# DSXiangLi/ChineseNER

Hardware: AMD Instinct MI355X
Metric: training samples/sec, bert_bilstm_crf (BERT-base + BiLSTM + CRF), msra-shaped (higher is better)
Workload: dtype bf16; 1 GPU; model=bert_bilstm_crf, global_batch=64, seq_len=128, parallelism=dp1

## Files before the change

### chinesener_amd/ops/functional.py

```python
from __future__ import annotations

import math
import os
from typing import Optional, Tuple

import torch
import torch.nn.functional as F

from . import reference as ref
from . import hip_enabled, get_ext


def _pad_last(t: torch.Tensor, target: int) -> torch.Tensor:
    d = t.shape[-1]
    return t if d == target else F.pad(t, (0, target - d))


class _LayerNormFn(torch.autograd.Function):
    @staticmethod
    def forward(ctx, x, weight, bias, eps):
        y, mean, rstd = get_ext().layernorm_fwd(x, weight, bias, eps)
        ctx.save_for_backward(x, weight, mean, rstd)
        return y

    @staticmethod
    def backward(ctx, dy):
        x, weight, mean, rstd = ctx.saved_tensors
        dx, dw, db = get_ext().layernorm_bwd(dy.contiguous(), x, weight, mean, rstd)
        return dx, dw, db, None


def layernorm(x, weight, bias, eps: float = 1e-12):
    if hip_enabled(x):
        shape = x.shape
        y = _LayerNormFn.apply(x.reshape(-1, shape[-1]).contiguous(), weight, bias, eps)
        return y.reshape(shape)
    return ref.layernorm(x, weight, bias, eps)


class _AddLayerNormFn(torch.autograd.Function):
    @staticmethod
    def forward(ctx, x, residual, weight, bias, eps):
        y, s, mean, rstd = get_ext().add_layernorm_fwd(x, residual, weight, bias, eps)
        ctx.save_for_backward(s, weight, mean, rstd)
        return y

    @staticmethod
    def backward(ctx, dy):
        s, weight, mean, rstd = ctx.saved_tensors
        dx, dw, db = get_ext().layernorm_bwd(dy.contiguous(), s, weight, mean, rstd)
        return dx, dx, dw, db, None


_rng_counter = None


def _rng_counter_for(device):
    global _rng_counter
    if _rng_counter is None or _rng_counter.device != device:
        seed = torch.initial_seed() & 0x7FFFFFFF
        _rng_counter = torch.tensor([seed], dtype=torch.int64, device=device)
    return _rng_counter


class _DropoutAddLNFn(torch.autograd.Function):

    @staticmethod
    def forward(ctx, x, res, weight, bias, eps, keep):
        y, s, mask, mean, rstd = get_ext().dropout_add_ln_fwd(
            x, res, weight, bias, eps, keep,
            _rng_counter_for(x.device))
        ctx.save_for_backward(s, weight, mask, mean, rstd)
        ctx.keep = keep
        return y

    @staticmethod
    def backward(ctx, dy):
        s, weight, mask, mean, rstd = ctx.saved_tensors
        dsum, dx, dw, db, _ = get_ext().dropout_add_ln_bwd(
            dy.contiguous(), s, weight, mean, rstd, mask, ctx.keep, False)
        return dx, dsum, dw, db, None, None


def dropout_add_layernorm(x, residual, weight, bias, eps: float = 1e-12,
                          p: float = 0.1, training: bool = True):
    if (training and p > 0 and hip_enabled(x) and x.dtype == torch.bfloat16
            and os.environ.get("CHINESENER_NO_FUSED_DROPOUT") != "1"):
        shape = x.shape
        y = _DropoutAddLNFn.apply(
            x.reshape(-1, shape[-1]).contiguous(),
            residual.to(x.dtype).reshape(-1, shape[-1]).contiguous(),
            weight, bias, eps, 1.0 - p)
        return y.reshape(shape)
    if training and p > 0:
        x = F.dropout(x, p, training)
    return add_layernorm(x, residual, weight, bias, eps)


def add_layernorm(x, residual, weight, bias, eps: float = 1e-12):
    if hip_enabled(x):
        shape = x.shape
        y = _AddLayerNormFn.apply(
            x.reshape(-1, shape[-1]).contiguous(),
            residual.to(x.dtype).reshape(-1, shape[-1]).contiguous(),
            weight, bias, eps)
        return y.reshape(shape)
    return ref.add_layernorm(x, residual, weight, bias, eps)


_GEMM_NT_CHOICE: dict = {}
_GEMM_NT_CALLS: dict = {}
_PICK_MIN_RECUR = 6


def _gemm_nt_mode() -> str:
    return os.environ.get("CHINESENER_GEMM_NT", "auto")


def _gemm_nt_ok(x2, w):
    return (x2.shape[0] % 128 == 0 and w.shape[0] % 128 == 0
            and w.shape[1] % 64 == 0 and x2.dtype == torch.bfloat16
            and w.dtype == torch.bfloat16)


def _tuning_active() -> bool:
    try:
        import torch.cuda.tunable as tun
        return tun.is_enabled() and tun.tuning_is_enabled()
    except Exception:
        return False


def _med_time(fn):
    import time as _time
    fn(); fn()
    torch.cuda.synchronize()
    ts = []
    for _ in range(3):
        t0 = _time.perf_counter()
        for _i in range(8):
            fn()
        torch.cuda.synchronize()
        ts.append((_time.perf_counter() - t0) / 8)
    return sorted(ts)[1]


def _pick2(key, fn_ours, fn_lib, min_recur: int = _PICK_MIN_RECUR) -> bool:
    hit = _GEMM_NT_CHOICE.get(key)
    if hit is not None:
        return hit
    if torch.cuda.is_current_stream_capturing() or _tuning_active():
        return False
    n = _GEMM_NT_CALLS.get(key, 0) + 1
    _GEMM_NT_CALLS[key] = n
    if n < min_recur:
        return False

    t_ours, t_lib = _med_time(fn_ours), _med_time(fn_lib)
    _GEMM_NT_CHOICE[key] = bool(t_ours <= t_lib)
    if os.environ.get("CHINESENER_GEMM_DEBUG") == "1":
        import sys
        print(f"[gemm-dispatch] {key}: ours {t_ours*1e6:.1f}us "
              f"lib {t_lib*1e6:.1f}us -> "
              f"{'ours' if _GEMM_NT_CHOICE[key] else 'lib'}",
              file=sys.stderr, flush=True)
    return _GEMM_NT_CHOICE[key]


def _pick_gemm_nt(x2, w, b) -> bool:
    key = (x2.shape[0], w.shape[0], w.shape[1], b is not None)
    hit = _GEMM_NT_CHOICE.get(key)
    if hit is not None:
        return hit
    if torch.cuda.is_current_stream_capturing() or _tuning_active():
        return False
    n = _GEMM_NT_CALLS.get(key, 0) + 1
    _GEMM_NT_CALLS[key] = n
    if n < _PICK_MIN_RECUR:
        return False
    ext = get_ext()

    t_ours = _med_time(lambda: ext.gemm_nt(x2, w, b, False))
    t_lib = _med_time(lambda: F.linear(x2, w, b))
    _GEMM_NT_CHOICE[key] = bool(t_ours <= t_lib)
    if os.environ.get("CHINESENER_GEMM_DEBUG") == "1":
        import sys
        print(f"[gemm-dispatch] fwd {key}: ours {t_ours*1e6:.1f}us "
              f"lib {t_lib*1e6:.1f}us -> "
              f"{'ours' if _GEMM_NT_CHOICE[key] else 'lib'}",
              file=sys.stderr, flush=True)
    return _GEMM_NT_CHOICE[key]


def _linear_fwd(x, w, b):
    mode = _gemm_nt_mode()
    if mode != "off":
        x2 = x.reshape(-1, x.shape[-1])
        if _gemm_nt_ok(x2, w):
            x2 = x2.contiguous()
            wc = w.contiguous()
            if mode == "force" or _pick_gemm_nt(x2, wc, b):
                y = get_ext().gemm_nt(x2, wc, b, False)
                return y.reshape(*x.shape[:-1], w.shape[0])
    return F.linear(x, w, b)


def _linear_dgrad(dyf, x, w):
    M, N = dyf.shape
    K = x.shape[-1]
    mode = _gemm_nt_mode()
    bf16 = (dyf.dtype == torch.bfloat16 and x.dtype == torch.bfloat16
            and w.dtype == torch.bfloat16)

    def dx_ours():
        return get_ext().gemm_nn(dyf.contiguous(), w.contiguous(), False)

    def dx_lib():
        return dyf @ w.to(dyf.dtype)

    if (mode != "off" and bf16 and M % 128 == 0 and K % 128 == 0
            and N % 64 == 0
            and (mode == "force"
                 or _pick2(("dx", M, N, K), dx_ours, dx_lib))):
        return dx_ours().reshape(x.shape)
    return dx_lib().reshape(x.shape)


def _linear_wgrad(dyf, x, w):
    M, N = dyf.shape
    K = x.shape[-1]
    x2 = x.reshape(-1, K)
    mode = _gemm_nt_mode()
    bf16 = dyf.dtype == torch.bfloat16 and x.dtype == torch.bfloat16

    def dw_ours():
        return get_ext().gemm_tn(dyf.contiguous(), x2.contiguous(), 0, False)

    def dw_lib():
        return dyf.T @ x2

    if (mode != "off" and bf16 and N % 128 == 0 and K % 128 == 0
            and M % 64 == 0
            and (mode == "force"
                 or _pick2(("dw", M, N, K), dw_ours, dw_lib))):
        return dw_ours().to(w.dtype)
    return dw_lib().to(w.dtype)


class _LinearFn(torch.autograd.Function):

    @staticmethod
    def forward(ctx, x, w, b):
        ctx.save_for_backward(x, w)
        ctx.has_bias = b is not None
        return _linear_fwd(x, w, b)

    @staticmethod
    def backward(ctx, dy):
        x, w = ctx.saved_tensors
        dyf = dy.reshape(-1, w.shape[0]).contiguous()
        dx = _linear_dgrad(dyf, x, w)
        dw = _linear_wgrad(dyf, x, w)
        db = get_ext().colsum(dyf) if ctx.has_bias else None
        return dx, dw, db


def linear(x, weight, bias=None):
    if (hip_enabled(x) and x.dtype == weight.dtype
            and not torch.is_autocast_enabled()):
        return _LinearFn.apply(x, weight,
                               bias.to(x.dtype) if bias is not None else None)
    return F.linear(x, weight, bias)


class _LinearDropoutAddLNFn(torch.autograd.Function):

    @staticmethod
    def forward(ctx, x, w, b, res, ln_w, ln_b, eps, keep):
        a = _linear_fwd(x, w, b)
        y, s, mask, mean, rstd = get_ext().dropout_add_ln_fwd(
            a.reshape(-1, a.shape[-1]).contiguous(), res, ln_w, ln_b, eps,
            keep, _rng_counter_for(x.device))
        ctx.save_for_backward(x, w, s, ln_w, mask, mean, rstd)
        ctx.keep = keep
        ctx.has_bias = b is not None
        return y

    @staticmethod
    def backward(ctx, dy):
        x, w, s, ln_w, mask, mean, rstd = ctx.saved_tensors
        dsum, dx_drop, dw_ln, db_ln, dbias = get_ext().dropout_add_ln_bwd(
            dy.contiguous(), s, ln_w, mean, rstd, mask, ctx.keep,
            ctx.has_bias)
        dx = _linear_dgrad(dx_drop, x, w)
        dw = _linear_wgrad(dx_drop, x, w)
        return dx, dw, dbias, dsum, dw_ln, db_ln, None, None


def linear_dropout_add_layernorm(x, weight, bias, residual, ln_w, ln_b,
                                 eps: float = 1e-12, p: float = 0.1,
                                 training: bool = True):
    if (training and p > 0 and hip_enabled(x) and x.dtype == torch.bfloat16
            and weight.dtype == x.dtype
            and (bias is None or bias.dtype == x.dtype)
            and os.environ.get("CHINESENER_NO_FUSED_DROPOUT") != "1"
            and not torch.is_autocast_enabled()):
        H = weight.shape[0]
        y = _LinearDropoutAddLNFn.apply(
            x, weight, bias,
            residual.to(x.dtype).reshape(-1, H).contiguous(),
            ln_w, ln_b, eps, 1.0 - p)
        return y.reshape(*x.shape[:-1], H)
    return dropout_add_layernorm(linear(x, weight, bias), residual, ln_w,
                                 ln_b, eps, p, training)


class _Embed3Fn(torch.autograd.Function):

    @staticmethod
    def forward(ctx, word_w, pos_w, tok_w, token_ids, segment_ids):
        ctx.save_for_backward(token_ids, segment_ids)
        ctx.shapes = (word_w.shape, pos_w.shape, tok_w.shape)
        return get_ext().embed3_fwd(word_w, pos_w, tok_w,
                                    token_ids.contiguous(),
                                    segment_ids.contiguous())

    @staticmethod
    def backward(ctx, dy):
        token_ids, segment_ids = ctx.saved_tensors
        (vs, ps, ts) = ctx.shapes
        B, L, H = dy.shape
        dyf = dy.reshape(-1, H).float()
        dw = torch.zeros(vs, dtype=torch.float32, device=dy.device)
        dw.index_add_(0, token_ids.reshape(-1), dyf)
        dw[0].zero_()
        dp = torch.zeros(ps, dtype=torch.float32, device=dy.device)
        dp[:L] = dy.float().sum(0)
        dt = torch.zeros(ts, dtype=torch.float32, device=dy.device)
        dt.index_add_(0, segment_ids.reshape(-1), dyf)
        return (dw.to(dy.dtype), dp.to(dy.dtype), dt.to(dy.dtype),
                None, None)


def embed3(word_w, pos_w, tok_w, token_ids, segment_ids):
    if (os.environ.get("CHINESENER_NO_EMBED3") != "1"
            and hip_enabled(word_w) and word_w.dtype == torch.bfloat16
            and word_w.shape[1] % 8 == 0
            and token_ids.shape[1] <= pos_w.shape[0]):
        return _Embed3Fn.apply(word_w, pos_w, tok_w, token_ids, segment_ids)
    pos = torch.arange(token_ids.shape[1], device=token_ids.device)
    return (F.embedding(token_ids, word_w, padding_idx=0) + pos_w[pos]
            + F.embedding(segment_ids, tok_w))


class _BiasGeluFn(torch.autograd.Function):
    @staticmethod
    def forward(ctx, x, bias):
        y = get_ext().bias_gelu_fwd(x, bias)
        ctx.save_for_backward(x, bias)
        return y

    @staticmethod
    def backward(ctx, dy):
        x, bias = ctx.saved_tensors
        dx, dbias = get_ext().bias_gelu_bwd(dy.contiguous(), x, bias)
        return dx, dbias


def bias_gelu(x, bias):
    if bias is not None and hip_enabled(x):
        shape = x.shape
        y = _BiasGeluFn.apply(x.reshape(-1, shape[-1]).contiguous(), bias)
        return y.reshape(shape)
    return ref.bias_gelu(x, bias)


def _fused_gelu_mode() -> str:
    return os.environ.get("CHINESENER_FUSED_GELU", "auto")


def _inner_decided(key) -> bool:
    return _gemm_nt_mode() != "auto" or key in _GEMM_NT_CHOICE


def _pick_fused(key, inner_key, fn_fused, fn_pair) -> bool:
    mode = _fused_gelu_mode()
    if mode != "auto":
        return mode == "force"
    if key not in _GEMM_NT_CHOICE and not _inner_decided(inner_key):
        return False
    return _pick2(key, fn_fused, fn_pair, min_recur=1)


def _ffn_up(x2, w1, b1, save_pre: bool):
    ext = get_ext()
    M, K = x2.shape
    N = w1.shape[0]

    def fused():
        return ext.gemm_nt_bias_gelu(x2, w1, b1, save_pre)

    def pair():
        u = _linear_fwd(x2, w1, None)
        return u, ext.bias_gelu_fwd(u, b1)

    key = ("ffn_up_gelu" if save_pre else "ffn_up_gelu_nopre", M, N, K)
    if _pick_fused(key, (M, N, K, False), fused, pair):
        u, g = fused()
        return u, g
    return pair()


def _ffn_dn(dx_drop, w2, u, b1):
    ext = get_ext()
    M, N = dx_drop.shape
    K = w2.shape[1]

    def fused():
        return ext.gemm_nn_dgelu(dx_drop, w2, u, b1)

    def pair():
        return ext.bias_gelu_bwd(_linear_dgrad(dx_drop, u, w2), u, b1)

    if _pick_fused(("ffn_dn_dgelu", M, N, K), ("dx", M, N, K), fused, pair):
        du, db1 = fused()
        return du, db1
    du, db1 = pair()
    return du, db1


class _FfnGeluFn(torch.autograd.Function):

    @staticmethod
    def forward(ctx, x, w1, b1, w2, b2, res, ln_w, ln_b, eps, keep):
        x2 = x.reshape(-1, x.shape[-1])
        u, g = _ffn_up(x2, w1, b1, True)
        a = _linear_fwd(g, w2, b2)
        y, s, mask, mean, rstd = get_ext().dropout_add_ln_fwd(
            a, res, ln_w, ln_b, eps, keep, _rng_counter_for(x.device))
        ctx.save_for_backward(x, w1, b1, w2, u, g, s, ln_w, mask, mean, rstd)
        ctx.keep = keep
        ctx.has_bias = b2 is not None
        return y

    @staticmethod
    def backward(ctx, dy):
        x, w1, b1, w2, u, g, s, ln_w, mask, mean, rstd = ctx.saved_tensors
        dsum, dx_drop, dw_ln, db_ln, db2 = get_ext().dropout_add_ln_bwd(
            dy.contiguous(), s, ln_w, mean, rstd, mask, ctx.keep,
            ctx.has_bias)
        dw2 = _linear_wgrad(dx_drop, g, w2)
        du, db1 = _ffn_dn(dx_drop, w2, u, b1)
        dw1 = _linear_wgrad(du, x, w1)
        dx = _linear_dgrad(du, x, w1)
        return dx, dw1, db1, dw2, db2, dsum, dw_ln, db_ln, None, None


def _ffn_fusable(x, w1, b1, w2, b2) -> bool:
    if not (hip_enabled(x) and _fused_gelu_mode() != "off"
            and not torch.is_autocast_enabled()):
        return False
    M = x.numel() // x.shape[-1] if x.shape[-1] else 0
    return (x.dtype == torch.bfloat16 and w1.dtype == x.dtype
            and w2.dtype == x.dtype and x.is_contiguous()
            and w1.is_contiguous() and w2.is_contiguous()
            and b1 is not None and b1.is_contiguous()
            and b1.dtype in (torch.bfloat16, torch.float32)
            and (b2 is None or b2.dtype == x.dtype)
            and M > 0 and M % 128 == 0 and w1.shape[0] % 128 == 0
            and w1.shape[1] % 128 == 0 and w2.shape[0] == w1.shape[1]
            and w2.shape[1] == w1.shape[0])


def ffn_gelu_dropout_add_layernorm(x, w1, b1, w2, b2, residual, ln_w, ln_b,
                                   eps: float = 1e-12, p: float = 0.1,
                                   training: bool = True):
    if _ffn_fusable(x, w1, b1, w2, b2):
        if (training and p > 0 and torch.is_grad_enabled()
                and os.environ.get("CHINESENER_NO_FUSED_DROPOUT") != "1"):
            H = w2.shape[0]
            y = _FfnGeluFn.apply(
                x, w1, b1, w2, b2,
                residual.to(x.dtype).reshape(-1, H).contiguous(),
                ln_w, ln_b, eps, 1.0 - p)
            return y.reshape(*x.shape[:-1], H)
        if not torch.is_grad_enabled():
            _, f = _ffn_up(x.reshape(-1, x.shape[-1]), w1, b1, False)
            return linear_dropout_add_layernorm(
                f.reshape(*x.shape[:-1], w1.shape[0]), w2, b2, residual,
                ln_w, ln_b, eps, p, training)
    f = bias_gelu(linear(x, w1), b1)
    return linear_dropout_add_layernorm(f, w2, b2, residual, ln_w, ln_b,
                                        eps, p, training)


def _attn_path(L: int, D: int, dtype, on_gpu: bool) -> str:
    if not on_gpu or dtype != torch.bfloat16 or D > 64 or L < 1:
        return "torch"
    mode = os.environ.get("CHINESENER_ATTN_TILED", "")
    if mode == "force":
        return "tiled" if L <= 512 else "torch"
    if ((L + 31) // 32) * 32 <= 176:
        return "lds"
    if mode != "off" and L <= 512:
        return "tiled"
    return "torch"


class _AttentionFn(torch.autograd.Function):
    @staticmethod
    def forward(ctx, q, k, v, lens, scale, tiled=False):
        ext = get_ext()
        fwd = ext.attn_tiled_fwd if tiled else ext.attn_fwd
        out, lse = fwd(q, k, v, lens, scale, 1.0, None)
        ctx.save_for_backward(q, k, v, out, lse, lens)
        ctx.scale = scale
        ctx.tiled = tiled
        return out

    @staticmethod
    def backward(ctx, dout):
        q, k, v, out, lse, lens = ctx.saved_tensors
        ext = get_ext()
        bwd = ext.attn_tiled_bwd if ctx.tiled else ext.attn_bwd
        dq, dk, dv = bwd(dout.contiguous(), q, k, v, out, lse, lens,
                         ctx.scale, 1.0, None)
        return dq, dk, dv, None, None, None


def attention(q, k, v, mask: Optional[torch.Tensor] = None,
              scale: Optional[float] = None, lens: Optional[torch.Tensor] = None):
    D = q.shape[-1]
    if scale is None:
        scale = 1.0 / math.sqrt(D)
    path = _attn_path(q.shape[2], D, q.dtype, hip_enabled(q))
    if path != "torch":
        Dp = 32 if D <= 32 else 64
        if lens is None:
            lens = (mask.long().sum(1) if mask is not None
                    else torch.full((q.shape[0],), q.shape[2],
                                    dtype=torch.long, device=q.device))
        out = _AttentionFn.apply(_pad_last(q, Dp).contiguous(),
                                 _pad_last(k, Dp).contiguous(),
                                 _pad_last(v, Dp).contiguous(),
                                 lens.to(torch.int32), float(scale),
                                 path == "tiled")
        return out[..., :D] if Dp != D else out
    return ref.attention(q, k, v, mask, scale)


class _AttentionQkvFn(torch.autograd.Function):

    @staticmethod
    def forward(ctx, qkv, lens, scale, keep, tiled=False):
        seed = None
        if keep < 1.0:
            ctr = _rng_counter_for(qkv.device)
            seed = ctr.clone()
            get_ext().bump_counter(ctr)
        ext = get_ext()
        fwd = ext.attn_tiled_fwd_qkv if tiled else ext.attn_fwd_qkv
        out, lse = fwd(qkv, lens, scale, keep, seed)
        ctx.save_for_backward(qkv, out, lse, lens,
                              seed if seed is not None
                              else torch.zeros(0))
        ctx.scale = scale
        ctx.keep = keep
        ctx.tiled = tiled
        return out

    @staticmethod
    def backward(ctx, dout):
        qkv, out, lse, lens, seed = ctx.saved_tensors
        ext = get_ext()
        bwd = ext.attn_tiled_bwd_qkv if ctx.tiled else ext.attn_bwd_qkv
        (dqkv,) = bwd(dout.contiguous(), qkv, out, lse, lens, ctx.scale,
                      ctx.keep, seed if seed.numel() else None)
        return dqkv, None, None, None, None


def attention_qkv(qkv, mask: Optional[torch.Tensor] = None,
                  lens: Optional[torch.Tensor] = None,
                  scale: Optional[float] = None,
                  p_drop: float = 0.0, training: bool = False):
    B, L, _, H, D = qkv.shape
    if scale is None:
        scale = 1.0 / math.sqrt(D)
    keep = 1.0 - p_drop if (training and p_drop > 0) else 1.0
    if os.environ.get("CHINESENER_NO_ATTN_DROP") == "1":
        keep = 1.0
    path = (_attn_path(L, D, qkv.dtype, hip_enabled(qkv))
            if D in (32, 64) else "torch")
    if path != "torch":
        if lens is None:
            lens = (mask.long().sum(1) if mask is not None
                    else torch.full((B,), L, dtype=torch.long,
                                    device=qkv.device))
        return _AttentionQkvFn.apply(qkv.contiguous(), lens.to(torch.int32),
                                     float(scale), float(keep),
                                     path == "tiled")
    q, k, v = (qkv[:, :, i].transpose(1, 2) for i in range(3))
    if keep < 1.0:
        out = ref.attention(q, k, v, mask, scale, p_drop=p_drop,
                            training=training)
    else:
        out = attention(q, k, v, mask=mask, scale=scale, lens=lens)
    return out.transpose(1, 2)


class _LinearAttentionQkvFn(torch.autograd.Function):

    @staticmethod
    def forward(ctx, x, w, b, lens, n_heads, scale, keep):
        B, L = x.shape[0], x.shape[1]
        qkv = _linear_fwd(x, w, b).reshape(B, L, 3, n_heads, -1).contiguous()
        seed = None
        if keep < 1.0:
            ctr = _rng_counter_for(x.device)
            seed = ctr.clone()
            get_ext().bump_counter(ctr)
        out, lse = get_ext().attn_fwd_qkv(qkv, lens, scale, keep, seed)
        ctx.save_for_backward(x, w, b, qkv, out, lse, lens,
                              seed if seed is not None else torch.zeros(0))
        ctx.scale = scale
        ctx.keep = keep
        return out

    @staticmethod
    def backward(ctx, dout):
        x, w, b, qkv, out, lse, lens, seed = ctx.saved_tensors
        dqkv, dbias = get_ext().attn_bwd_qkv_dbias(
            dout.contiguous(), qkv, out, lse, lens, ctx.scale, ctx.keep,
            seed if seed.numel() else None, b)
        dyf = dqkv.reshape(-1, w.shape[0])
        dx = _linear_dgrad(dyf, x, w)
        dw = _linear_wgrad(dyf, x, w)
        return dx, dw, dbias, None, None, None, None


def linear_attention_qkv(x, weight, bias, n_heads: int,
                         mask: Optional[torch.Tensor] = None,
                         lens: Optional[torch.Tensor] = None,
                         p_drop: float = 0.0, training: bool = False):
    B, L = x.shape[0], x.shape[1]
# ... 326 lines not shown
```

### csrc/bindings.cpp

```cpp
#include <torch/extension.h>

#include <vector>

std::vector<at::Tensor> layernorm_fwd(const at::Tensor&, const at::Tensor&,
                                      const at::Tensor&, double);
std::vector<at::Tensor> add_layernorm_fwd(const at::Tensor&, const at::Tensor&,
                                          const at::Tensor&, const at::Tensor&,
                                          double);
std::vector<at::Tensor> layernorm_bwd(const at::Tensor&, const at::Tensor&,
                                      const at::Tensor&, const at::Tensor&,
                                      const at::Tensor&);
at::Tensor bias_gelu_fwd(const at::Tensor&, const at::Tensor&);
std::vector<at::Tensor> bias_gelu_bwd(const at::Tensor&, const at::Tensor&,
                                      const at::Tensor&);
std::vector<at::Tensor> masked_ce_fwd(const at::Tensor&, const at::Tensor&,
                                      const at::Tensor&);
at::Tensor masked_ce_bwd(const at::Tensor&, const at::Tensor&,
                         const at::Tensor&, const at::Tensor&,
                         const at::Tensor&);
at::Tensor colsum(const at::Tensor&);
std::vector<at::Tensor> dropout_add_ln_fwd(const at::Tensor&,
                                           const at::Tensor&,
                                           const at::Tensor&,
                                           const at::Tensor&, double, double,
                                           const at::Tensor&);
at::Tensor mask_scale(const at::Tensor&, const at::Tensor&, double);
std::vector<at::Tensor> dropout_add_ln_bwd(const at::Tensor&,
                                           const at::Tensor&,
                                           const at::Tensor&,
                                           const at::Tensor&,
                                           const at::Tensor&,
                                           const at::Tensor&, double, bool);
void bump_counter(const at::Tensor&);
at::Tensor wgrad(const at::Tensor&, const at::Tensor&, long);
at::Tensor wgrad2(const at::Tensor&, const at::Tensor&, long);
at::Tensor gemm_nt(const at::Tensor&, const at::Tensor&,
                   c10::optional<at::Tensor>, bool);
at::Tensor gemm_tn(const at::Tensor&, const at::Tensor&, long, bool);
at::Tensor gemm_nn(const at::Tensor&, const at::Tensor&, bool);
std::vector<at::Tensor> gemm_nt_bias_gelu(const at::Tensor&,
                                          const at::Tensor&,
                                          const at::Tensor&, bool);
std::vector<at::Tensor> gemm_nn_dgelu(const at::Tensor&, const at::Tensor&,
                                      const at::Tensor&, const at::Tensor&);
at::Tensor embed3_fwd(const at::Tensor&, const at::Tensor&,
                      const at::Tensor&, const at::Tensor&,
                      const at::Tensor&);
std::vector<at::Tensor> crf_fwd(const at::Tensor&, const at::Tensor&,
                                const at::Tensor&, const at::Tensor&);
at::Tensor crf_viterbi(const at::Tensor&, const at::Tensor&,
                       const at::Tensor&);
std::vector<at::Tensor> crf_wide_fwd(const at::Tensor&, const at::Tensor&,
                                     const at::Tensor&, const at::Tensor&);
at::Tensor crf_wide_viterbi(const at::Tensor&, const at::Tensor&,
                            const at::Tensor&);
std::vector<at::Tensor> crf_path_posterior(const at::Tensor&,
                                           const at::Tensor&,
                                           const at::Tensor&,
                                           const at::Tensor&);
std::vector<at::Tensor> crf_nbest(const at::Tensor&, const at::Tensor&,
                                  const at::Tensor&, int64_t);
std::vector<int64_t> crf_nbest_route(int64_t, int64_t, int64_t);
at::Tensor softlexicon_fwd(const at::Tensor&, const at::Tensor&,
                           const at::Tensor&);
std::vector<at::Tensor> softlexicon_bwd(const at::Tensor&, const at::Tensor&,
                                        const at::Tensor&, const at::Tensor&);
void multi_tensor_adamw(std::vector<at::Tensor>, std::vector<at::Tensor>,
                        std::vector<at::Tensor>, std::vector<at::Tensor>,
                        std::vector<at::Tensor>, std::vector<double>,
                        std::vector<double>, double, double, double,
                        c10::optional<at::Tensor>);
at::Tensor multi_tensor_sumsq(std::vector<at::Tensor>);
void multi_tensor_scale(std::vector<at::Tensor>, const at::Tensor&);
std::vector<at::Tensor> adamw_build_meta(
    std::vector<at::Tensor>, std::vector<at::Tensor>, std::vector<at::Tensor>,
    std::vector<at::Tensor>, std::vector<at::Tensor>, std::vector<double>,
    std::vector<double>);
void multi_tensor_adamw_run(const at::Tensor&, long, long, bool, double,
                            double, double, c10::optional<at::Tensor>);
std::vector<at::Tensor> norm_build_meta(std::vector<at::Tensor>);
at::Tensor multi_tensor_sumsq_run(const at::Tensor&, long, const at::Tensor&);
void multi_tensor_scale_run(const at::Tensor&, long, const at::Tensor&);
void multi_tensor_adamw_tab_run(const at::Tensor&, long, long, bool,
                                std::vector<at::Tensor>,
                                std::vector<c10::optional<at::Tensor>>, double,
                                double, double, c10::optional<at::Tensor>,
                                c10::optional<at::Tensor>);
long grad_table_slots();
long sumsq_chunk_elems();
at::Tensor sumsq_build_chunks(std::vector<long>, std::vector<long>,
                              const at::Tensor&);
at::Tensor multi_tensor_sumsq_coef_run(const at::Tensor&, std::vector<long>,
                                       std::vector<long>,
                                       std::vector<c10::optional<at::Tensor>>,
                                       double);
std::vector<at::Tensor> attn_fwd(const at::Tensor&, const at::Tensor&,
                                 const at::Tensor&, const at::Tensor&, double,
                                 double, c10::optional<at::Tensor>);
std::vector<at::Tensor> attn_bwd(const at::Tensor&, const at::Tensor&,
                                 const at::Tensor&, const at::Tensor&,
                                 const at::Tensor&, const at::Tensor&,
                                 const at::Tensor&, double, double,
                                 c10::optional<at::Tensor>);
std::vector<at::Tensor> attn_fwd_qkv(const at::Tensor&, const at::Tensor&,
                                     double, double,
                                     c10::optional<at::Tensor>);
std::vector<at::Tensor> attn_bwd_qkv(const at::Tensor&, const at::Tensor&,
                                     const at::Tensor&, const at::Tensor&,
                                     const at::Tensor&, double, double,
                                     c10::optional<at::Tensor>);
std::vector<at::Tensor> attn_bwd_qkv_dbias(
    const at::Tensor&, const at::Tensor&, const at::Tensor&,
    const at::Tensor&, const at::Tensor&, double, double,
    c10::optional<at::Tensor>, const at::Tensor&);
std::vector<at::Tensor> attn_tiled_fwd(const at::Tensor&, const at::Tensor&,
                                       const at::Tensor&, const at::Tensor&,
                                       double, double,
                                       c10::optional<at::Tensor>);
std::vector<at::Tensor> attn_tiled_bwd(const at::Tensor&, const at::Tensor&,
                                       const at::Tensor&, const at::Tensor&,
                                       const at::Tensor&, const at::Tensor&,
                                       const at::Tensor&, double, double,
                                       c10::optional<at::Tensor>);
std::vector<at::Tensor> attn_tiled_fwd_qkv(const at::Tensor&,
                                           const at::Tensor&, double, double,
                                           c10::optional<at::Tensor>);
std::vector<at::Tensor> attn_tiled_bwd_qkv(const at::Tensor&,
                                           const at::Tensor&,
                                           const at::Tensor&,
                                           const at::Tensor&,
                                           const at::Tensor&, double, double,
                                           c10::optional<at::Tensor>);
std::vector<at::Tensor> tener_attn_fwd(const at::Tensor&, const at::Tensor&,
                                       const at::Tensor&, const at::Tensor&,
                                       const at::Tensor&, const at::Tensor&);
std::vector<at::Tensor> tener_attn_bwd(const at::Tensor&, const at::Tensor&,
                                       const at::Tensor&, const at::Tensor&,
                                       const at::Tensor&, const at::Tensor&,
                                       const at::Tensor&, const at::Tensor&,
                                       const at::Tensor&);
at::Tensor mfma_probe(const at::Tensor&, const at::Tensor&);
std::vector<at::Tensor> lstm_fwd(const at::Tensor&, const at::Tensor&,
                                 const at::Tensor&, bool, bool);
std::vector<at::Tensor> lstm_bwd(const at::Tensor&, const at::Tensor&,
                                 const at::Tensor&, const at::Tensor&,
                                 const at::Tensor&, const at::Tensor&, bool,
                                 bool);
std::vector<at::Tensor> bilstm_fwd_l(const at::Tensor&, const at::Tensor&,
                                     const at::Tensor&, bool, double);
at::Tensor bilstm_bwd_l(const at::Tensor&, const at::Tensor&,
                        const at::Tensor&, const at::Tensor&,
                        const at::Tensor&, bool, double);

PYBIND11_MODULE(_hip_ops, m) {
  m.doc() = "chinesener_amd gfx950 HIP kernels";
  m.def("layernorm_fwd", &layernorm_fwd);
  m.def("add_layernorm_fwd", &add_layernorm_fwd);
  m.def("layernorm_bwd", &layernorm_bwd);
  m.def("bias_gelu_fwd", &bias_gelu_fwd);
  m.def("bias_gelu_bwd", &bias_gelu_bwd);
  m.def("masked_ce_fwd", &masked_ce_fwd);
  m.def("masked_ce_bwd", &masked_ce_bwd);
  m.def("colsum", &colsum);
  m.def("dropout_add_ln_fwd", &dropout_add_ln_fwd);
  m.def("mask_scale", &mask_scale);
  m.def("dropout_add_ln_bwd", &dropout_add_ln_bwd);
  m.def("bump_counter", &bump_counter);
  m.def("wgrad", &wgrad);
  m.def("wgrad2", &wgrad2);
  m.def("gemm_nt", &gemm_nt, py::arg("a"), py::arg("b"),
        py::arg("bias") = c10::nullopt, py::arg("fp32_out") = false);
  m.def("gemm_tn", &gemm_tn, py::arg("a"), py::arg("b"),
        py::arg("split") = 0, py::arg("fp32_out") = false);
  m.def("gemm_nn", &gemm_nn, py::arg("a"), py::arg("b"),
        py::arg("fp32_out") = false);
  m.def("gemm_nt_bias_gelu", &gemm_nt_bias_gelu, py::arg("a"), py::arg("b"),
        py::arg("bias"), py::arg("save_pre") = true);
  m.def("gemm_nn_dgelu", &gemm_nn_dgelu, py::arg("a"), py::arg("b"),
        py::arg("u"), py::arg("bias"));
  m.def("embed3_fwd", &embed3_fwd);
  m.def("crf_fwd", &crf_fwd);
  m.def("crf_viterbi", &crf_viterbi);
  m.def("crf_path_posterior", &crf_path_posterior, py::arg("emissions"),
        py::arg("lens"), py::arg("transitions"), py::arg("path"));
  m.def("crf_nbest", &crf_nbest, py::arg("emissions"), py::arg("lens"),
        py::arg("transitions"), py::arg("k"));
  m.def("crf_nbest_route", &crf_nbest_route, py::arg("seq_len"),
        py::arg("label_size"), py::arg("k"));
  m.def("softlexicon_fwd", &softlexicon_fwd);
  m.def("softlexicon_bwd", &softlexicon_bwd);
  m.def("multi_tensor_adamw", &multi_tensor_adamw);
  m.def("multi_tensor_sumsq", &multi_tensor_sumsq);
  m.def("multi_tensor_scale", &multi_tensor_scale);
  m.def("adamw_build_meta", &adamw_build_meta);
  m.def("multi_tensor_adamw_run", &multi_tensor_adamw_run);
  m.def("norm_build_meta", &norm_build_meta);
  m.def("multi_tensor_sumsq_run", &multi_tensor_sumsq_run);
  m.def("multi_tensor_scale_run", &multi_tensor_scale_run);
  m.def("multi_tensor_adamw_tab_run", &multi_tensor_adamw_tab_run);
  m.def("sumsq_build_chunks", &sumsq_build_chunks);
  m.def("multi_tensor_sumsq_coef_run", &multi_tensor_sumsq_coef_run);
  m.def("grad_table_slots", &grad_table_slots);
  m.def("sumsq_chunk_elems", &sumsq_chunk_elems);
  m.def("attn_fwd", &attn_fwd);
  m.def("attn_bwd", &attn_bwd);
  m.def("attn_fwd_qkv", &attn_fwd_qkv);
  m.def("attn_bwd_qkv", &attn_bwd_qkv);
  m.def("attn_bwd_qkv_dbias", &attn_bwd_qkv_dbias);
  m.def("attn_tiled_fwd", &attn_tiled_fwd);
  m.def("attn_tiled_bwd", &attn_tiled_bwd);
  m.def("attn_tiled_fwd_qkv", &attn_tiled_fwd_qkv);
  m.def("attn_tiled_bwd_qkv", &attn_tiled_bwd_qkv);
  m.def("tener_attn_fwd", &tener_attn_fwd);
  m.def("tener_attn_bwd", &tener_attn_bwd);
  m.def("mfma_probe", &mfma_probe);
  m.def("lstm_fwd", &lstm_fwd);
  m.def("lstm_bwd", &lstm_bwd);
  m.def("bilstm_fwd", &bilstm_fwd_l);
  m.def("bilstm_bwd", &bilstm_bwd_l);
}
```

### csrc/embed.hip

```cpp
#include "common.h"

__global__ __launch_bounds__(256) void embed3_kernel(
    const bf16* __restrict__ word,
    const bf16* __restrict__ pos,
    const bf16* __restrict__ tok,
    const long* __restrict__ ids,
    const long* __restrict__ segs,
    bf16* __restrict__ out,
    long R, int H, int L) {
  const long row = blockIdx.x;
  if (row >= R) return;
  const long wrow = ids[row];
  const long srow = segs[row];
  const int prow = (int)(row % L);
  const bf16* w = word + wrow * H;
  const bf16* p = pos + (long)prow * H;
  const bf16* s = tok + srow * H;
  bf16* o = out + row * H;
  for (int c = threadIdx.x * 8; c < H; c += blockDim.x * 8) {
    const bf16x8 wv = *reinterpret_cast<const bf16x8*>(w + c);
    const bf16x8 pv = *reinterpret_cast<const bf16x8*>(p + c);
    const bf16x8 sv = *reinterpret_cast<const bf16x8*>(s + c);
    bf16x8 ov;
#pragma unroll
    for (int e = 0; e < 8; ++e)
      ov[e] = (__bf16)((float)wv[e] + (float)pv[e] + (float)sv[e]);
    *reinterpret_cast<bf16x8*>(o + c) = ov;
  }
}

at::Tensor embed3_fwd(const at::Tensor& word, const at::Tensor& pos,
                      const at::Tensor& tok, const at::Tensor& token_ids,
                      const at::Tensor& segment_ids) {
  CHECK_CUDA_CONTIG(word);
  CHECK_CUDA_CONTIG(pos);
  CHECK_CUDA_CONTIG(tok);
  CHECK_CUDA_CONTIG(token_ids);
  CHECK_CUDA_CONTIG(segment_ids);
  TORCH_CHECK(word.scalar_type() == at::kBFloat16 &&
                  pos.scalar_type() == at::kBFloat16 &&
                  tok.scalar_type() == at::kBFloat16,
              "embed3: bf16 tables");
  const int H = word.size(1);
  TORCH_CHECK(H % 8 == 0, "embed3: hidden % 8");
  const long B = token_ids.size(0), L = token_ids.size(1);
  const long R = B * L;
  auto out = at::empty({B, L, (long)H}, word.options());
  hipLaunchKernelGGL(embed3_kernel, dim3((unsigned)R), dim3(256), 0,
                     cur_stream(word), (const bf16*)word.data_ptr(),
                     (const bf16*)pos.data_ptr(), (const bf16*)tok.data_ptr(),
                     token_ids.data_ptr<long>(), segment_ids.data_ptr<long>(),
                     (bf16*)out.data_ptr(), R, H, (int)L);
  HIP_CHECK_LAST();
  return out;
}
```

Before: 5428 samples/sec.

## Replace embedding backward index_add with sorted-index segmented-sum HIP kernels

Replaces the PyTorch embedding backward (fp32 zeros, index_add_ scatter, then bf16 casts) with a custom path. It builds a sorted row index by token id through a counting-rank sort, then writes each vocab row's gradient directly with a per-row gather-sum. Heavy tokens are split into chunks and reduced in a second pass. Position and segment gradients are computed in one column-reduction kernel. This avoids atomics, the fp32 vocab-sized buffer and the extra casts, at the cost of several more kernel launches and an O(R²/slices) ranking step.

```diff
diff --git a/chinesener_amd/ops/functional.py b/chinesener_amd/ops/functional.py
--- a/chinesener_amd/ops/functional.py
+++ b/chinesener_amd/ops/functional.py
@@ -315,6 +315,30 @@
                                  ln_b, eps, p, training)
 
 
+def _embed3_bwd_torch(dy, token_ids, segment_ids, vs, ps, ts):
+    B, L, H = dy.shape
+    dyf = dy.reshape(-1, H).float()
+    dw = torch.zeros(vs, dtype=torch.float32, device=dy.device)
+    dw.index_add_(0, token_ids.reshape(-1), dyf)
+    dw[0].zero_()
+    dp = torch.zeros(ps, dtype=torch.float32, device=dy.device)
+    dp[:L] = dy.float().sum(0)
+    dt = torch.zeros(ts, dtype=torch.float32, device=dy.device)
+    dt.index_add_(0, segment_ids.reshape(-1), dyf)
+    return dw.to(dy.dtype), dp.to(dy.dtype), dt.to(dy.dtype)
+
+
+def _embed3_bwd_eligible(dy, vs, ts) -> bool:
+    if os.environ.get("CHINESENER_EMBED3_BWD") == "off":
+        return False
+    _, seg_cap, max_rows, max_keys = get_ext().embed3_bwd_limits()
+    B, L, H = dy.shape
+    R = B * L
+    return (dy.dtype == torch.bfloat16 and H % 8 == 0
+            and 1 <= ts[0] <= seg_cap and 1 <= R <= max_rows
+            and vs[0] * R <= max_keys)
+
+
 class _Embed3Fn(torch.autograd.Function):
 
     @staticmethod
@@ -329,17 +353,14 @@
     def backward(ctx, dy):
         token_ids, segment_ids = ctx.saved_tensors
         (vs, ps, ts) = ctx.shapes
-        B, L, H = dy.shape
-        dyf = dy.reshape(-1, H).float()
-        dw = torch.zeros(vs, dtype=torch.float32, device=dy.device)
-        dw.index_add_(0, token_ids.reshape(-1), dyf)
-        dw[0].zero_()
-        dp = torch.zeros(ps, dtype=torch.float32, device=dy.device)
-        dp[:L] = dy.float().sum(0)
-        dt = torch.zeros(ts, dtype=torch.float32, device=dy.device)
-        dt.index_add_(0, segment_ids.reshape(-1), dyf)
-        return (dw.to(dy.dtype), dp.to(dy.dtype), dt.to(dy.dtype),
-                None, None)
+        if _embed3_bwd_eligible(dy, vs, ts):
+            dw, dp, dt = get_ext().embed3_bwd(
+                dy.contiguous(), token_ids.contiguous(),
+                segment_ids.contiguous(), vs[0], ps[0], ts[0])
+        else:
+            dw, dp, dt = _embed3_bwd_torch(dy, token_ids, segment_ids,
+                                           vs, ps, ts)
+        return dw, dp, dt, None, None
 
 
 def embed3(word_w, pos_w, tok_w, token_ids, segment_ids):
diff --git a/csrc/bindings.cpp b/csrc/bindings.cpp
--- a/csrc/bindings.cpp
+++ b/csrc/bindings.cpp
@@ -46,6 +46,9 @@
 at::Tensor embed3_fwd(const at::Tensor&, const at::Tensor&,
                       const at::Tensor&, const at::Tensor&,
                       const at::Tensor&);
+std::vector<at::Tensor> embed3_bwd(const at::Tensor&, const at::Tensor&,
+                                   const at::Tensor&, long, long, long);
+std::vector<long> embed3_bwd_limits();
 std::vector<at::Tensor> crf_fwd(const at::Tensor&, const at::Tensor&,
                                 const at::Tensor&, const at::Tensor&);
 at::Tensor crf_viterbi(const at::Tensor&, const at::Tensor&,
@@ -179,6 +182,9 @@
   m.def("gemm_nn_dgelu", &gemm_nn_dgelu, py::arg("a"), py::arg("b"),
         py::arg("u"), py::arg("bias"));
   m.def("embed3_fwd", &embed3_fwd);
+  m.def("embed3_bwd", &embed3_bwd, py::arg("dy"), py::arg("token_ids"),
+        py::arg("segment_ids"), py::arg("V"), py::arg("P"), py::arg("S"));
+  m.def("embed3_bwd_limits", &embed3_bwd_limits);
   m.def("crf_fwd", &crf_fwd);
   m.def("crf_viterbi", &crf_viterbi);
   m.def("crf_path_posterior", &crf_path_posterior, py::arg("emissions"),
diff --git a/csrc/embed.hip b/csrc/embed.hip
--- a/csrc/embed.hip
+++ b/csrc/embed.hip
@@ -1,4 +1,6 @@
 #include "common.h"
+#include "slab_colsum.h"
+#include "sorted_index.h"
 
 __global__ __launch_bounds__(256) void embed3_kernel(
     const bf16* __restrict__ word,
@@ -54,3 +56,277 @@
   HIP_CHECK_LAST();
   return out;
 }
+
+#define EB_CHUNK 16
+#define EB_INFLIGHT 8
+#define EB_SEG_CAP 8
+#define EB_BSLICES 8
+#define EB_COLVECS 32
+
+template <bool PARTIAL>
+__device__ __forceinline__ void eb_sum_rows(
+    const bf16* __restrict__ dy, const int* __restrict__ order, int s, int e,
+    int H, int lane, bf16* __restrict__ out_b, float* __restrict__ out_f) {
+  for (int c = lane * 8; c < H; c += WAVE * 8) {
+    float acc[8];
+#pragma unroll
+    for (int k = 0; k < 8; ++k) acc[k] = 0.f;
+    for (int p = s; p < e; p += EB_INFLIGHT) {
+      bf16x8 x[EB_INFLIGHT];
+#pragma unroll
+      for (int u = 0; u < EB_INFLIGHT; ++u) {
+        if (p + u < e) {
+          const long r = order[p + u];
+          x[u] = *reinterpret_cast<const bf16x8*>(dy + r * H + c);
+        } else {
+#pragma unroll
+          for (int k = 0; k < 8; ++k) x[u][k] = (__bf16)0.f;
+        }
+      }
+#pragma unroll
+      for (int u = 0; u < EB_INFLIGHT; ++u)
+#pragma unroll
+        for (int k = 0; k < 8; ++k) acc[k] += (float)x[u][k];
+    }
+    if (PARTIAL) {
+      f32x4 lo = {acc[0], acc[1], acc[2], acc[3]};
+      f32x4 hi = {acc[4], acc[5], acc[6], acc[7]};
+      *reinterpret_cast<f32x4*>(out_f + c) = lo;
+      *reinterpret_cast<f32x4*>(out_f + c + 4) = hi;
+    } else {
+      bf16x8 ov;
+#pragma unroll
+      for (int k = 0; k < 8; ++k) ov[k] = (__bf16)acc[k];
+      *reinterpret_cast<bf16x8*>(out_b + c) = ov;
+    }
+  }
+}
+
+struct EbChunk {
+  int v, k, m, s, n;
+};
+__device__ __forceinline__ bool eb_slot_chunk(const int* __restrict__ skey,
+                                              const int* __restrict__ start,
+                                              int j, EbChunk* ch) {
+  const int v = skey[(j + 1) * EB_CHUNK - 1];
+  if (v == 0) return false;
+  const int s = start[v];
+  const int n = start[v + 1] - s;
+  const int m = n / EB_CHUNK;
+  const int k = j - s / EB_CHUNK;
+  if (m < 2 || k < 0 || k >= m) return false;
+  ch->v = v; ch->k = k; ch->m = m; ch->s = s; ch->n = n;
+  return true;
+}
+
+__global__ __launch_bounds__(256) void embed3_bwd_word_kernel(
+    const bf16* __restrict__ dy, const int* __restrict__ order,
+    const int* __restrict__ skey, const int* __restrict__ start,
+    bf16* __restrict__ dw, float* __restrict__ slab, int V, int H,
+    int nslot) {
+  const int lane = threadIdx.x & (WAVE - 1);
+  const int w = blockIdx.x * 4 + threadIdx.x / WAVE;
+  if (w < V) {
+    const int s = start[w];
+    const int n = start[w + 1] - s;
+    bf16* o = dw + (long)w * H;
+    if (w == 0 || n == 0) {
+      bf16x8 z;
+#pragma unroll
+      for (int k = 0; k < 8; ++k) z[k] = (__bf16)0.f;
+      for (int c = lane * 8; c < H; c += WAVE * 8)
+        *reinterpret_cast<bf16x8*>(o + c) = z;
+    } else if (n < 2 * EB_CHUNK) {
+      eb_sum_rows<false>(dy, order, s, s + n, H, lane, o, nullptr);
+    }
+  } else if (w - V < nslot) {
+    const int j = w - V;
+    EbChunk ch;
+    if (!eb_slot_chunk(skey, start, j, &ch)) return;
+    const int cs = ch.s + (int)((long)ch.k * ch.n / ch.m);
+    const int ce = ch.s + (int)((long)(ch.k + 1) * ch.n / ch.m);
+    eb_sum_rows<true>(dy, order, cs, ce, H, lane, nullptr,
+                      slab + (long)j * H);
+  }
+}
+
+__global__ __launch_bounds__(EB_COLVECS * EB_BSLICES) void embed3_bwd_word_finish_kernel(
+    const float* __restrict__ slab, const int* __restrict__ skey,
+    const int* __restrict__ start, bf16* __restrict__ dw, int H) {
+  __shared__ float red[EB_BSLICES][EB_COLVECS][9];
+  const int j = blockIdx.x;
+  EbChunk ch;
+  if (!eb_slot_chunk(skey, start, j, &ch) || ch.k != 0) return;
+  const int tx = threadIdx.x % EB_COLVECS;
+  const int ty = threadIdx.x / EB_COLVECS;
+  const int c = (blockIdx.y * EB_COLVECS + tx) * 8;
+  const bool live = c < H;
+  float acc[8];
+#pragma unroll
+  for (int k = 0; k < 8; ++k) acc[k] = 0.f;
+  if (live) {
+    const float* p = slab + (long)j * H + c;
+#pragma unroll 4
+    for (int q = ty; q < ch.m; q += EB_BSLICES) {
+      const f32x4 lo = *reinterpret_cast<const f32x4*>(p + (long)q * H);
+      const f32x4 hi = *reinterpret_cast<const f32x4*>(p + (long)q * H + 4);
+#pragma unroll
+      for (int k = 0; k < 4; ++k) {
+        acc[k] += lo[k];
+        acc[4 + k] += hi[k];
+      }
+    }
+  }
+#pragma unroll
+  for (int k = 0; k < 8; ++k) red[ty][tx][k] = acc[k];
+  __syncthreads();
+  if (ty == 0 && live) {
+    bf16x8 ov;
+#pragma unroll
+    for (int k = 0; k < 8; ++k) {
+      float a = red[0][tx][k];
+#pragma unroll
+      for (int y = 1; y < EB_BSLICES; ++y) a += red[y][tx][k];
+      ov[k] = (__bf16)a;
+    }
+    *reinterpret_cast<bf16x8*>(dw + (long)ch.v * H + c) = ov;
+  }
+}
+
+__global__ __launch_bounds__(EB_COLVECS * EB_BSLICES) void embed3_bwd_pos_seg_kernel(
+    const bf16* __restrict__ dy, const long* __restrict__ segs,
+    bf16* __restrict__ dp, float* __restrict__ slab, int B, int L, int H,
+    int S) {
+  __shared__ float red[EB_BSLICES][EB_COLVECS][9];
+  const int tx = threadIdx.x % EB_COLVECS;
+  const int ty = threadIdx.x / EB_COLVECS;
+  const int l = blockIdx.x;
+  const int c = (blockIdx.y * EB_COLVECS + tx) * 8;
+  const bool live = c < H;
+  if (l >= L) {
+    if (live && ty == 0) {
+      bf16x8 z;
+#pragma unroll
+      for (int k = 0; k < 8; ++k) z[k] = (__bf16)0.f;
+      *reinterpret_cast<bf16x8*>(dp + (long)l * H + c) = z;
+    }
+    return;
+  }
+  float acc[EB_SEG_CAP + 1][8];
+#pragma unroll
+  for (int q = 0; q <= EB_SEG_CAP; ++q)
+#pragma unroll
+    for (int k = 0; k < 8; ++k) acc[q][k] = 0.f;
+  if (live) {
+#pragma unroll 4
+    for (int b = ty; b < B; b += EB_BSLICES) {
+      const long r = (long)b * L + l;
+      const bf16x8 x = *reinterpret_cast<const bf16x8*>(dy + r * H + c);
+      const long seg = segs[r];
+#pragma unroll
+      for (int k = 0; k < 8; ++k) acc[0][k] += (float)x[k];
+#pragma unroll
+      for (int q = 0; q < EB_SEG_CAP; ++q)
+        if (q < S && seg == q) {
+#pragma unroll
+          for (int k = 0; k < 8; ++k) acc[q + 1][k] += (float)x[k];
+        }
+    }
+  }
+#pragma unroll
+  for (int q = 0; q <= EB_SEG_CAP; ++q) {
+    if (q <= S) {
+      __syncthreads();
+#pragma unroll
+      for (int k = 0; k < 8; ++k) red[ty][tx][k] = acc[q][k];
+      __syncthreads();
+      if (ty == 0 && live) {
+        float a[8];
+#pragma unroll
+        for (int k = 0; k < 8; ++k) a[k] = red[0][tx][k];
+#pragma unroll
+        for (int y = 1; y < EB_BSLICES; ++y)
+#pragma unroll
+          for (int k = 0; k < 8; ++k) a[k] += red[y][tx][k];
+        if (q == 0) {
+          bf16x8 ov;
+#pragma unroll
+          for (int k = 0; k < 8; ++k) ov[k] = (__bf16)a[k];
+          *reinterpret_cast<bf16x8*>(dp + (long)l * H + c) = ov;
+        } else {
+          float* o = slab + ((long)l * S + (q - 1)) * H + c;
+          f32x4 lo = {a[0], a[1], a[2], a[3]};
+          f32x4 hi = {a[4], a[5], a[6], a[7]};
+          *reinterpret_cast<f32x4*>(o) = lo;
+          *reinterpret_cast<f32x4*>(o + 4) = hi;
+        }
+      }
+    }
+  }
+}
+
+std::vector<long> embed3_bwd_limits() {
+  return {EB_CHUNK, EB_SEG_CAP, SIDX_MAX_ROWS, SIDX_MAX_KEYS};
+}
+
+static bool embed3_bwd_supported(long R, long V, long H, long S) {
+  return H >= 8 && H % 8 == 0 && S >= 1 && S <= EB_SEG_CAP &&
+         sidx_supported(R, V);
+}
+
+std::vector<at::Tensor> embed3_bwd(const at::Tensor& dy,
+                                   const at::Tensor& token_ids,
+                                   const at::Tensor& segment_ids, long V,
+                                   long P, long S) {
+  CHECK_CUDA_CONTIG(dy);
+  CHECK_CUDA_CONTIG(token_ids);
+  CHECK_CUDA_CONTIG(segment_ids);
+  TORCH_CHECK(dy.scalar_type() == at::kBFloat16 && dy.dim() == 3,
+              "embed3_bwd: dy [B, L, H] bf16");
+  TORCH_CHECK(token_ids.scalar_type() == at::kLong &&
+                  segment_ids.scalar_type() == at::kLong,
+              "embed3_bwd: int64 ids");
+  const long B = dy.size(0), L = dy.size(1), H = dy.size(2);
+  const long R = B * L;
+  TORCH_CHECK(token_ids.numel() == R && segment_ids.numel() == R,
+              "embed3_bwd: ids [B, L]");
+  TORCH_CHECK(L <= P, "embed3_bwd: L <= P");
+  TORCH_CHECK(embed3_bwd_supported(R, V, H, S),
+              "embed3_bwd: need H % 8 == 0, S <= ", EB_SEG_CAP, ", B*L <= ",
+              SIDX_MAX_ROWS, " and V*B*L <= 2^32");
+  hipStream_t stream = cur_stream(dy);
+  auto dw = at::empty({V, H}, dy.options());
+  auto dp = at::empty({P, H}, dy.options());
+  auto dt = at::empty({S, H}, dy.options());
+  const bf16* dyp = (const bf16*)dy.data_ptr();
+
+  SortedIndex si = build_sorted_index(token_ids, R, V, stream);
+  const int nslot = (int)(R / EB_CHUNK);
+  auto wslab = at::empty({std::max(nslot, 1), H},
+                         dy.options().dtype(at::kFloat));
+  hipLaunchKernelGGL(embed3_bwd_word_kernel,
+                     dim3((unsigned)((V + nslot + 3) / 4)), dim3(256), 0,
+                     stream, dyp, si.order, si.skey, si.start,
+                     (bf16*)dw.data_ptr(), wslab.data_ptr<float>(), (int)V,
+                     (int)H, nslot);
+  if (nslot > 0)
+    hipLaunchKernelGGL(
+        embed3_bwd_word_finish_kernel,
+        dim3((unsigned)nslot,
+             (unsigned)((H + 8 * EB_COLVECS - 1) / (8 * EB_COLVECS))),
+        dim3(EB_COLVECS * EB_BSLICES), 0, stream,
+                       (const float*)wslab.data_ptr<float>(), si.skey,
+                       si.start, (bf16*)dw.data_ptr(), (int)H);
+
+  auto tslab = at::empty({L, S * H}, dy.options().dtype(at::kFloat));
+  hipLaunchKernelGGL(
+      embed3_bwd_pos_seg_kernel,
+      dim3((unsigned)P, (unsigned)((H + 8 * EB_COLVECS - 1) / (8 * EB_COLVECS))),
+      dim3(EB_COLVECS * EB_BSLICES), 0, stream, dyp,
+      segment_ids.data_ptr<long>(), (bf16*)dp.data_ptr(),
+      tslab.data_ptr<float>(), (int)B, (int)L, (int)H, (int)S);
+  launch_slab_colsum<bf16, bf16>(tslab, dt.data_ptr(), (int)(S * H),
+                                 dt.data_ptr(), stream);
+  HIP_CHECK_LAST();
+  return {dw, dp, dt};
+}
diff --git a/csrc/sorted_index.h b/csrc/sorted_index.h
--- /dev/null
+++ b/csrc/sorted_index.h
@@ -0,0 +1,118 @@
+#pragma once
+
+#include "common.h"
+
+#define SIDX_MAX_ROWS 32768
+#define SIDX_MAX_KEYS (1l << 32)
+#define SIDX_TILE 256
+#define SIDX_SLICE_MAX 2048
+
+static inline bool sidx_supported(long R, long V) {
+  return R >= 1 && V >= 1 && R <= SIDX_MAX_ROWS &&
+         R * V <= SIDX_MAX_KEYS;
+}
+
+__device__ __forceinline__ int sidx_id(const long* __restrict__ ids, int r,
+                                       int V) {
+  const long id = ids[r];
+  return (id < 0 || id >= V) ? 0 : (int)id;
+}
+
+__device__ __forceinline__ unsigned sidx_key(const long* __restrict__ ids,
+                                             int r, int R, int V) {
+  return (unsigned)sidx_id(ids, r, V) * (unsigned)R + (unsigned)r;
+}
+
+__global__ __launch_bounds__(SIDX_TILE) void sidx_count_kernel(
+    const long* __restrict__ ids, int R, int V, int SL,
+    int* __restrict__ cnt) {
+  __shared__ __attribute__((aligned(16))) unsigned keys[SIDX_SLICE_MAX];
+  const int j0 = blockIdx.y * SL;
+  for (int j = threadIdx.x; j < SL; j += SIDX_TILE) {
+    const int rr = j0 + j;
+    keys[j] = rr < R ? sidx_key(ids, rr, R, V) : 0xFFFFFFFFu;
+  }
+  __syncthreads();
+  const int r = blockIdx.x * SIDX_TILE + threadIdx.x;
+  if (r >= R) return;
+  const unsigned ki = sidx_key(ids, r, R, V);
+  int c = 0;
+#pragma unroll 4
+  for (int j = 0; j < SL; j += 4) {
+    const uint4 k = *reinterpret_cast<const uint4*>(&keys[j]);
+    c += (int)(k.x < ki) + (int)(k.y < ki) + (int)(k.z < ki) +
+         (int)(k.w < ki);
+  }
+  cnt[(long)blockIdx.y * R + r] = c;
+}
+
+__global__ __launch_bounds__(256) void sidx_place_kernel(
+    const long* __restrict__ ids, int R, int V, int NS,
+    const int* __restrict__ cnt, int* __restrict__ order,
+    int* __restrict__ skey) {
+  const int r = blockIdx.x * 256 + threadIdx.x;
+  if (r >= R) return;
+  int pos = 0;
+  for (int y = 0; y < NS; ++y) pos += cnt[(long)y * R + r];
+  if (pos < R) {
+    order[pos] = r;
+    skey[pos] = sidx_id(ids, r, V);
+  }
+}
+
+__global__ __launch_bounds__(256) void sidx_start_kernel(
+    const int* __restrict__ skey, int R, int V, int* __restrict__ start) {
+  const int p = blockIdx.x * 256 + threadIdx.x;
+  const int lane = threadIdx.x & (WAVE - 1);
+  int a = 0, b = 0;
+  if (p <= R) {
+    a = p > 0 ? skey[p - 1] + 1 : 0;
+    b = p < R ? skey[p] + 1 : V + 1;
+  }
+  const bool wide = b - a > 8;
+  if (!wide)
+    for (int v = a; v < b; ++v) start[v] = p;
+  unsigned long long todo = __ballot(wide);
+  while (todo) {
+    const int src = __ffsll((long long)todo) - 1;
+    todo &= todo - 1;
+    const int aa = __shfl(a, src), bb = __shfl(b, src), pp = __shfl(p, src);
+    for (int v = aa + lane; v < bb; v += WAVE) start[v] = pp;
+  }
+}
+
+struct SortedIndex {
+  at::Tensor buf;
+  const int* order;
+  const int* skey;
+  const int* start;
+};
+
+static inline SortedIndex build_sorted_index(const at::Tensor& ids, long R,
+                                             long V, hipStream_t stream) {
+  TORCH_CHECK(sidx_supported(R, V), "sorted index: need 1 <= R <= ",
+              SIDX_MAX_ROWS, " and V * R <= 2^32, got R = ", R, ", V = ", V);
+  const int SL = R <= 8192 ? 512 : SIDX_SLICE_MAX;
+  const int NS = (int)((R + SL - 1) / SL);
+  SortedIndex si;
+  si.buf = at::empty({(long)NS * R + 2 * R + V + 1},
+                     ids.options().dtype(at::kInt));
+  int* cnt = si.buf.data_ptr<int>();
+  int* order = cnt + (long)NS * R;
+  int* skey = order + R;
+  int* start = skey + R;
+  const long* idp = ids.data_ptr<long>();
+  hipLaunchKernelGGL(sidx_count_kernel,
+                     dim3((unsigned)((R + SIDX_TILE - 1) / SIDX_TILE), NS),
+                     dim3(SIDX_TILE), 0, stream, idp, (int)R, (int)V, SL, cnt);
+  hipLaunchKernelGGL(sidx_place_kernel, dim3((unsigned)((R + 255) / 256)),
+                     dim3(256), 0, stream, idp, (int)R, (int)V, NS,
+                     (const int*)cnt, order, skey);
+  hipLaunchKernelGGL(sidx_start_kernel, dim3((unsigned)((R + 1 + 255) / 256)),
+                     dim3(256), 0, stream, (const int*)skey, (int)R, (int)V,
+                     start);
+  si.order = order;
+  si.skey = skey;
+  si.start = start;
+  return si;
+}
```

New measurement: 5557 samples/sec (median of 6 runs). 1.02x the previous value.
